# slimgroup/SetIntersectionProjection.jl

Hardware: AMD Instinct MI355X
Metric: PARSDMM iterations/sec (higher is better)
Workload: dtype f32

## Files before the change

### setintersectionprojection.jl_amd/csrc/engine.cpp

```cpp
#include "engine.h"
#include "comm.h"
#include "device_memory.h"
#include "dist_dft.h"
#include "ext_proj.h"
#include "host_prefault.h"
#include "l21_joint.h"
#include "set_config.h"
#include "solve_rules.h"
#include "sparse_granules.h"

#include <algorithm>
#include <array>
#include <chrono>
#include <cmath>
#include <cstdio>
#include <cstdlib>
#include <cstring>
#include <limits>
#include <thread>
#include <exception>

namespace sipx {

const LaunchObserver*& launch_observer() {
// ... 1720 lines not shown
        B.in_rhs = behind ? 0 : 1;
      }
    }
    if (ma.nblk == 0) return false;
    return K<T>::yl_multi(stream_, G_, ma, true);
  }
  static bool sweep_eligible(const SetState<T>& s) {
    return s.owned && !s.custom && !s.ext_kind && !s.dist_ext &&
           (s.prox == PX_BOUNDS || s.prox == PX_L1 || s.prox == PX_PROX_L1 || s.prox == PX_L2 || s.prox == PX_ANNULUS || s.prox == PX_DIST);
  }

  void spec_fill(const LockStep& L, size_t j, long long fseg, long long rank_off, double cap_max, SpecPackArgs<T>& pk, SpecFinishArgs<T>& fa) {
    const SetState<T>& s = sets_[L.tp[j]];
    ProjScalars<T>* ps = L.feas_ps ? s.psf : s.ps;
    SpecPackSet<T>& P = pk.s[j];
    P.ps = ps; P.partials = s.ptmp; P.maxpart = s.mpart; P.compact = s.cbuf;
    P.seg = fbuf_ + rank_off + (long long)j * fseg;
    P.is_l1 = s.prox == PX_L1 ? 1 : 0;
    SpecFinishSet<T>& F = fa.s[j];
    F.ps = ps;
    F.da = DecideArgs{L.args[j].prox, (L.args[j].flags & F_NOSPEC) ? 1 : 0, (double)L.args[j].plo, (double)L.args[j].phi, cap_max, s.Mtrue};
    F.reg = stage_ + j * L.RS;
    F.fseg0 = fbuf_ + (long long)j * fseg;
    F.compact = s.cbuf; F.partials = s.ptmp; F.radius = L.args[j].phi;
    F.host_want = L.ctl[j].host_want; F.verdict = L.ctl[j].verdict;
  }

  void spec_exchange_searches(LockStep& L, int it) {
    const std::vector<int>& tp = L.tp;
    const long long fseg = hooks_.fcap + fast_hdr<T>();
    const long long fchunk = (long long)tp.size() * fseg;
    const unsigned seq = ++spec_seq_ & 0x3fffffffu;
    for (size_t j = 0; j < tp.size(); ++j) {
      L.ctl[j].verdict = (unsigned*)hverd_ + tp[j];
      L.ctl[j].seq = seq;
    }
    if ((int)tp.size() <= SPEC_MAX_SETS) {
      SpecPackArgs<T> pk;
      SpecFinishArgs<T> fa;
      pk.nsets = fa.nsets = (int)tp.size();
      pk.cap = hooks_.fcap;
      fa.world = comm_->world; fa.fchunk = fchunk; fa.seq = seq;
      if (!L.feas_ps && !L.v_is_s && Gr_.n[0] % 4 == 0) {
        LeanMulti<T> lm;
        lm.ns = 0;
        std::vector<size_t> who;
        for (size_t j = 0; j < tp.size() && lm.ns < LEAN_MAX; ++j) {
// ... 149 lines not shown
        LeanSet<T>& S = G.s[G.ns++];
        S.a = L.args[j]; S.a.ps = ps; S.ps = ps; S.compact = s.cbuf; S.partials = s.ptmp; S.maxpart = s.mpart;
      }
      return G;
    };
    std::vector<size_t> all(tp.size());
    for (size_t j = 0; j < tp.size(); ++j) all[j] = j;
    std::vector<size_t> l1s;
    for (size_t j = 0; vec && j < tp.size(); ++j)
      if (sets_[tp[j]].prox == PX_L1 && !(L.args[j].flags & F_NOSPEC)) l1s.push_back(j);
    for (size_t k = 0; k < l1s.size(); k += LEAN_MAX) K<T>::lean_multi(stream_, Gr_, group(l1s, k));
    if (vec && env_knobs().pass_multi) {
      for (size_t k = 0; k < all.size(); k += LEAN_MAX) K<T>::pass_multi(0, stream_, Gr_, group(all, k), L.v_is_s);
    } else {
      for (size_t j : l1s) {
        L.ctl[j].lean_done = 1;
        L.ctl[j].lean_known = feas_ps ? 0 : ((hlean_[tp[j]] >> 16) & 1);
      }
      for (size_t j = 0; j < tp.size(); ++j) search_stage(13, stream_, L, j);
    }
    SpecPackArgs<T> pk;
    SpecFinishArgs<T> fa;
    pk.nsets = fa.nsets = (int)tp.size();
    pk.local = fa.local = 1;
    pk.cap = 0;
    fa.world = 1; fa.fchunk = (long long)tp.size() * fseg; fa.seq = seq;
    for (size_t j = 0; j < tp.size(); ++j) spec_fill(L, j, fseg, 0, 0.0, pk, fa);
    K<T>::spec_sums_pack(stream_, pk);
    K<T>::spec_finish(stream_, fa);
    std::vector<size_t> fb;
    bool refine = false;
    for (size_t j = 0; j < tp.size(); ++j) {
      const unsigned w = wait_verdict(hverd_ + tp[j], seq);
      batch_searches_ += 1;
      if (!(w & 1u)) continue;
      batch_fallbacks_ += 1;
      if (env_knobs().trace_searches)
        std::fprintf(stderr, "[sipx search] search %lld (set %d%s): fallback%s\n", batch_searches_, tp[j], feas_ps ? ", feasibility" : "", (w & 2u) ? " with refinement" : "");
      fb.push_back(j);
      refine |= (w & 2u) != 0;
    }
    const bool spec_debug = env_knobs().spec_debug;
    if (spec_debug && !feas_ps) {
      std::fprintf(stderr, "[sipx spec] batched chain, search seq %u\n", seq);
      for (size_t j = 0; j < tp.size(); ++j) dump_ps(tp[j], stage_ + j * L.RS);
    }
    if (fb.empty()) return;
    auto tail = [&](int stage) {
      for (size_t j : fb) {
        SetState<T>& s = sets_[tp[j]];
        K<T>::search_tail(stage, stream_, L.args[j], feas_ps ? s.psf : s.ps, s.ptmp, s.mpart, s.cbuf, s.Mtrue, L.ctl[j], stage_ + j * L.RS);
// ... 1127 lines not shown
    }
    o += ", \"rank_route\": {\"calls\": " + std::to_string(rc[0]) + ", \"warm_started_subspace\": " + std::to_string(rc[1]) +
         ", \"full_decomposition\": " + std::to_string(rc[2]) + ", \"products_with_gram\": " + std::to_string(rc[3]) + "}";
    long long fc[4] = {0, 0, 0, 0};
    for (const auto& st : sets_) {
      if (!st.ext || st.ext_kind != EXT_L21_SEG) continue;
      long long c[4];
      st.ext->route_counts(c);
      fc[0] += c[0]; fc[1] = std::max(fc[1], c[1]); fc[3] += c[3];
    }
    o += ", \"l21_frames\": {\"passes_total\": " + std::to_string(fc[0]) + ", \"passes_max\": " + std::to_string(fc[1]) +
         ", \"frames\": " + std::to_string(fc[3]) + "}}";
    if (!peek) start_stats(enable);
    return o.c_str();
  }
  double stat_pair_overhead_ms() const { return stat_pair_ms_; }

  void debug_proj(int set, int which, double* o) override {
    need_final();
    for (int k = 0; k < 16; ++k) o[k] = 0;
    if (set < 0 || set >= p_n_) throw std::runtime_error("set index out of range");
    const ProjScalars<T>* d = (which & 1) ? sets_[set].psf : sets_[set].ps;
    if (!d) return;
    ProjScalars<T> h;
    SIPX_HIP(hipStreamSynchronize(stream_));
    SIPX_HIP(hipMemcpy(&h, d, sizeof(h), hipMemcpyDeviceToHost));
    o[0] = h.need; o[1] = h.theta; o[2] = h.theta_prev; o[3] = h.hw; o[4] = h.spec_lo; o[5] = h.spec_hi; o[6] = h.lo;
    o[7] = h.hi; o[8] = h.asum; o[9] = h.vmax; o[10] = h.dbg[0]; o[11] = h.dbg[1]; o[12] = h.dbg[2]; o[13] = h.dbg[3];
    o[14] = h.refine;
    o[15] = h.lean + 2 * h.dbg_sampled;
    if (which & 2) { o[4] = h.samp_theta; o[5] = h.samp_lo; o[6] = h.samp_hi; o[7] = h.samp_c; }
  }

  void* stream() override { return (void*)stream_; }
  void* dev_rhs() override { return rhs_; }
  void* dev_x() override { return x_; }
  void get_rhs(void* out) override {
    need_final();
    if (slab_local_ && comm_->world > 1) throw std::runtime_error("a slab-decomposed context holds its planes of rhs only");
    SIPX_HIP(hipStreamSynchronize(stream_));
    SIPX_HIP(hipMemcpy(out, rhs_, Nx_ * sizeof(T), hipMemcpyDeviceToHost));
  }

 private:
  struct KSample { int kid; double bytes_survey, bytes_moved; };
  struct KAgg { long long launches = 0, noops = 0; double ms = 0, bytes_survey = 0, bytes_moved = 0; };
// ... 658 lines not shown
  bool lean_multi_ = false;
  bool head_done_ = false;
  int merged_nslots_ = 0;
  int sums_flags_ = 0;
  volatile unsigned long long* ticket_ = nullptr;
  unsigned cg_seq_ = 0;
  bool slab_req_ = false, slab_ = false;
  hipStream_t fan_st_ = nullptr;
  hipEvent_t fan_fork_ = nullptr;
  double* fan_ptmp_ = nullptr;
  T *fan_mpart_ = nullptr, *fan_c_ = nullptr;
  long long fan_exchanges_ = 0;
  bool slab_loose_ = false;
  bool slab_full_req_ = false, slab_local_ = false;
  std::string selftest_ = "none", mapped_why_;
  double* agree_buf_ = nullptr;
  bool selftest_mapped_failed_ = false, selftest_alltoall_failed_ = false;
  std::string a2a_why_;
  long long wlo_ = 0, whi_ = 0;
  Grid Gr_, Gyl_;
  ChainHooks hooks_;
  T* gbuf_ = nullptr;
  double *stage_ = nullptr, *sstage_ = nullptr;
  const ChainHooks* hooks() const { return slab_ ? &hooks_ : nullptr; }
  double obj_ss_ = 0, evo_ss_ = 0, xx_ss_ = 0;
  bool have_log_sums_ = false;
  hipEvent_t cg_ev_[2] = {nullptr, nullptr};
  std::vector<hipEvent_t> stat_ev_;
  std::vector<KSample> samples_;
  std::vector<size_t> open_;
  int stats_mode_ = 0;
  LaunchObserver obs_{this, &Engine<T>::obs_begin, &Engine<T>::obs_end};
  std::string stats_json_;
  double stat_pair_ms_ = 0;
};

EngineBase* make_engine(int dtype, int ndim, const int64_t* n, const double* h, int device) {
  const int count = hip_device_count();
  if (device < 0 || device >= count) throw std::runtime_error("libsipx: device index out of range");
  if (dtype == SIPX_F32) return new Engine<float>(ndim, n, h, device);
  if (dtype == SIPX_F64) return new Engine<double>(ndim, n, h, device);
  throw std::runtime_error("dtype must be SIPX_F32 or SIPX_F64");
}

template <typename T>
static void cds_spmv_T(int64_t N, int d, const void* R, const int64_t* off, const void* x, void* y) {
// ... 99 lines not shown
```

### setintersectionprojection.jl_amd/csrc/kernels_proj.hip

```cpp
#include <cstdlib>
#include <cstring>
#include <stdexcept>
#include <string>
#include <type_traits>

#include "sipx_device.h"

namespace sipx {

#if defined(__HIP_DEVICE_COMPILE__) && !defined(__gfx950__)
#error "kernels_proj.hip: the relaxed-atomics hand-offs assume gfx950 (see the comment above); port them to release/acquire first"
#endif

constexpr double L1_CAP = 131072.0;
constexpr int L1_REFINES = 1;
constexpr int L1_REFINES_SLAB = 6;
#ifndef SIPX_SPEC_CAP
#define SIPX_SPEC_CAP 1024
#endif
constexpr int SPEC_CAP = SIPX_SPEC_CAP;
constexpr double L1_HW_MAX = 1e-2;
constexpr double L1_CAPDIV = 64.0;
constexpr int L1_WIN_LO = 3, L1_WIN_HI = 4;
__device__ __forceinline__ double l1_probe_mult(int k) {
// ... 1165 lines not shown
__device__ __forceinline__ DD dd_add(DD a, double b) {
  const double s = a.hi + b, bb = s - a.hi;
  const double e = (a.hi - (s - bb)) + (b - bb);
  return DD{s, a.lo + e};
}
__device__ __forceinline__ DD dd_add(DD a, DD b) {
  const double s = a.hi + b.hi, bb = s - a.hi;
  const double e = (a.hi - (s - bb)) + (b.hi - bb);
  const double lo = (a.lo + b.lo) + e;
  const double hi = s + lo;
  return DD{hi, lo - (hi - s)};
}
__device__ __forceinline__ double shfl_xor_f64(double v, int m) {
  const long long b = __double_as_longlong(v);
  const int lo = __shfl_xor((int)(b & 0xffffffffll), m, 64), hi = __shfl_xor((int)(b >> 32), m, 64);
  return __longlong_as_double(((long long)hi << 32) | (unsigned int)lo);
}
__device__ __forceinline__ DD wave_sum_dd(DD v) {
#pragma unroll
  for (int m = 1; m < 64; m <<= 1) v = dd_add(v, DD{shfl_xor_f64(v.hi, m), shfl_xor_f64(v.lo, m)});
  return v;
}

#ifndef SIPX_SOLVE_NT
#define SIPX_SOLVE_NT 1024
#endif
constexpr int SOLVE_G = 32;
constexpr long long SOLVE_COOP_MIN = 1ll << 17;
static_assert(SOLVE_G <= SIPX_SOLVE_SLOTS, "ProjScalars holds SIPX_SOLVE_SLOTS cooperative slots");

template <typename T>
__device__ void l1_solve_body(ProjScalars<T>* ps, T radius, const T* __restrict__ compact, const double* __restrict__ partials,
                              long long true_len, int* host_want, int only_if_settled,
                              const int G, const int wg) {
  constexpr int NT = SIPX_SOLVE_NT;
  if (only_if_settled && ps->need && !ps->spec_ok) return;
  __shared__ double ssum[NT / 64];
  __shared__ double ssum_lo[NT / 64];
  __shared__ double scnt[NT / 64];
  __shared__ double sh_theta, sh_sa, sh_ca;
  __shared__ int sh_done;
  const int need = ps->need;
  const long long n_all = need ? (long long)ps->n_compact : 0;
  const bool coop = G > 1 && n_all >= SOLVE_COOP_MIN;
  if (!coop && wg != 0) return;
  double theta = 0;
  int iters_done = 0;
  if (need) {
    if (ps->spec_ok) {
      if (threadIdx.x == 0) { sh_sa = ps->s_above; sh_ca = ps->c_above; }
    } else {
      double s = 0, c = 0;
      for (int i = threadIdx.x; i < NB; i += NT) {
        s += partials[(long long)SL_ABOVE_S * NB + i];
        c += partials[(long long)SL_ABOVE_C * NB + i];
      }
      s = wave_sum(s);
      c = wave_sum(c);
      if ((threadIdx.x & 63) == 0) { ssum[threadIdx.x >> 6] = s; scnt[threadIdx.x >> 6] = c; }
      __syncthreads();
      if (threadIdx.x == 0) {
        double S = 0, Cc = 0;
        for (int i = 0; i < NT / 64; ++i) { S += ssum[i]; Cc += scnt[i]; }
        sh_sa = S; sh_ca = Cc;
      }
    }
    __syncthreads();
    const long long nv_all = n_all / 4;
    const long long per = coop ? (nv_all + G - 1) / G : nv_all;
    const long long v0 = coop ? (long long)wg * per : 0, v1 = coop ? (v0 + per < nv_all ? v0 + per : nv_all) : nv_all;
    const bool tail_owner = !coop || wg == G - 1;
    const double sa = sh_sa, ca = sh_ca, b = (double)radius;
    theta = ps->lo;
    double cprev = -1;
    for (int it = 0; it < 200; ++it) {
      DD s = {0.0, 0.0};
      double c = 0;
      {
        const long long nv = v1;
        for (long long i0 = v0 + threadIdx.x; i0 < nv; i0 += 4 * NT) {
          Vec<T, 4> q[4];
#pragma unroll
          for (int u = 0; u < 4; ++u) {
            const long long i = i0 + (long long)u * NT;
            if (i < nv) q[u] = ldv_u<T, 4>(compact + 4 * i);
            else { q[u].v[0] = q[u].v[1] = q[u].v[2] = q[u].v[3] = T(0); }
          }
#pragma unroll
          for (int u = 0; u < 4; ++u)
#pragma unroll
            for (int k = 0; k < 4; ++k) {
              const double av = (double)q[u].v[k];
              if (av > theta) { s = dd_add(s, av); c += 1.0; }
            }
        }
        if (tail_owner)
          for (long long e = 4 * nv_all + threadIdx.x; e < n_all; e += NT) {
            const double av = (double)compact[e];
            if (av > theta) { s = dd_add(s, av); c += 1.0; }
          }
      }
      s = wave_sum_dd(s);
      c = wave_sum(c);
      __syncthreads();
      if ((threadIdx.x & 63) == 0) { ssum[threadIdx.x >> 6] = s.hi; ssum_lo[threadIdx.x >> 6] = s.lo; scnt[threadIdx.x >> 6] = c; }
      __syncthreads();
      if (threadIdx.x == 0) {
        DD Sd = {0.0, 0.0};
        double Cc = 0;
        for (int i = 0; i < NT / 64; ++i) { Sd = dd_add(Sd, DD{ssum[i], ssum_lo[i]}); Cc += scnt[i]; }
        if (coop) {
          const int buf = it & 1;
          __hip_atomic_store(&ps->coop_hi[buf][wg], Sd.hi, __ATOMIC_RELAXED, __HIP_MEMORY_SCOPE_AGENT);
          __hip_atomic_store(&ps->coop_lo[buf][wg], Sd.lo, __ATOMIC_RELAXED, __HIP_MEMORY_SCOPE_AGENT);
          __hip_atomic_store(&ps->coop_c[buf][wg], Cc, __ATOMIC_RELAXED, __HIP_MEMORY_SCOPE_AGENT);
          __hip_atomic_fetch_add(&ps->coop_arrive, 1u, __ATOMIC_RELEASE, __HIP_MEMORY_SCOPE_AGENT);
          const unsigned want = (unsigned)G * (unsigned)(it + 1);
          unsigned spins = 0;
          while (__hip_atomic_load(&ps->coop_arrive, __ATOMIC_ACQUIRE, __HIP_MEMORY_SCOPE_AGENT) < want) {
            if (__hip_atomic_load(&ps->coop_abort, __ATOMIC_RELAXED, __HIP_MEMORY_SCOPE_AGENT)) break;
            if (++spins > 8000000u) {
              __hip_atomic_store(&ps->coop_abort, 1u, __ATOMIC_RELAXED, __HIP_MEMORY_SCOPE_AGENT);
              break;
            }
            __builtin_amdgcn_s_sleep(4);
          }
          Sd = DD{0.0, 0.0};
          Cc = 0;
          for (int k = 0; k < G; ++k) {
            Sd = dd_add(Sd, DD{__hip_atomic_load(&ps->coop_hi[buf][k], __ATOMIC_RELAXED, __HIP_MEMORY_SCOPE_AGENT),
                               __hip_atomic_load(&ps->coop_lo[buf][k], __ATOMIC_RELAXED, __HIP_MEMORY_SCOPE_AGENT)});
            Cc += __hip_atomic_load(&ps->coop_c[buf][k], __ATOMIC_RELAXED, __HIP_MEMORY_SCOPE_AGENT);
          }
        }
        const double S = Sd.hi + Sd.lo;
        const double tot = ca + Cc;
        double tn = theta;
        if (tot > 0) tn = (sa + S - b) / tot;
        sh_done = (Cc == cprev || !(tot > 0)) ? 1 : 0;
        if (coop && __hip_atomic_load(&ps->coop_abort, __ATOMIC_RELAXED, __HIP_MEMORY_SCOPE_AGENT)) sh_done = 1;
        sh_theta = tn > theta ? tn : theta;
        sh_sa = sa; sh_ca = tot;
        scnt[0] = Cc;
      }
      __syncthreads();
      theta = sh_theta;
      cprev = scnt[0];
      iters_done = it + 1;
      if (sh_done) break;
    }
  }
  if (threadIdx.x == 0) {
    if (coop) {
      const unsigned t = __hip_atomic_fetch_add(&ps->coop_finish, 1u, __ATOMIC_ACQ_REL, __HIP_MEMORY_SCOPE_AGENT);
      if (t != (unsigned)G - 1u) return;
      ps->dbg[3] = ps->coop_abort ? -1.0 : 0.0;
      ps->coop_arrive = 0;
      ps->coop_finish = 0;
      ps->coop_abort = 0;
    }
    if (need) {
      if (sh_ca >= (double)true_len && true_len > 1) theta = (ps->asum - (double)ps->vmin - (double)radius) / (double)(true_len - 1);
      const T th = (T)theta;
      ps->theta = th > T(0) ? th : T(0);
      if (ps->gather_overflow) ps->theta = (T)NAN;
    }
    ps->dbg[0] = (double)ps->n_compact; ps->dbg[1] = ps->spec_overflow; ps->dbg[2] = ps->spec_ok;
    ps->dbg[3] = (coop && ps->dbg[3] < 0) ? -1.0 : (double)iters_done;
    ps->lean = (need && theta > 0 && ps->spec_ok && !ps->spec_overflow && sh_ca < (double)true_len) ? 1 : 0;
    ps->want_sample = 0;
    if (need && theta > 0) {
      double hw = ps->hw;
      if (!(ps->theta_prev > 0)) ps->want_sample = 1;
      if (ps->theta_prev > 0) {
        const double d = fabs(theta / ps->theta_prev - 1.0);
        ps->want_sample = (3.0 * d > L1_HW_MAX) ? 1 : 0;
        if (ps->rescaled) ps->resc_bad = d > L1_HW_MAX ? 1 : 0;
        hw = 3.0 * d;
        double hw_floor = 2e-3;
        if (ps->spec_ok && n_all > 0 && ps->hw > 0) {
          const double tgt = fmax(32768.0, (double)true_len / 1024.0);
          hw_floor = ps->hw * tgt / (double)n_all;
          hw_floor = hw_floor < 1e-3 ? 1e-3 : (hw_floor > 4e-3 ? 4e-3 : hw_floor);
        }
        hw = hw < hw_floor ? hw_floor : (hw > L1_HW_MAX ? L1_HW_MAX : hw);
        if (ps->spec_overflow) hw = ps->hw * 0.5;
      }
      ps->hw = hw;
      ps->theta_prev = theta;
      for (int k = 0; k < L1_K; ++k) ps->t[k] = (double)(T)(theta * (1.0 + hw * l1_probe_mult(k)));
      ps->spec_lo = ps->t[L1_WIN_LO];
      ps->spec_hi = ps->t[L1_WIN_HI];
    } else if (ps->theta_prev > 0) {
      for (int k = 0; k < L1_K; ++k) ps->t[k] = (double)(T)(ps->theta_prev * (1.0 + ps->hw * l1_probe_mult(k)));
      ps->spec_lo = ps->t[L1_WIN_LO];
      ps->spec_hi = ps->t[L1_WIN_HI];
    }
    ps->n_compact = 0;
    ps->spec_overflow = 0;
    if (ps->sampled && need && theta > 0) { ps->samp_bias = ps->samp_theta - theta; ps->samp_bias_ok = 1; }
    ps->dbg_sampled = ps->sampled;
    ps->sampled = 0;
    ps->rescaled = 0;
    if (host_want)
      __hip_atomic_store(host_want, ps->want_sample | (ps->rounds_used << 8) | ((ps->lean && ps->spec_hi > ps->spec_lo) ? (1 << 16) : 0), __ATOMIC_RELAXED,
                         __HIP_MEMORY_SCOPE_SYSTEM);
  }
}

template <typename T>
__global__ __launch_bounds__(SIPX_SOLVE_NT) void k_l1_solve(ProjScalars<T>* ps, T radius, const T* __restrict__ compact,
                                                   const double* __restrict__ partials, long long true_len, int* host_want, int only_if_settled) {
  l1_solve_body<T>(ps, radius, compact, partials, true_len, host_want, only_if_settled, (int)gridDim.x,
                   (int)blockIdx.x);
}

constexpr double CARD_CAP = 8192.0;
constexpr int CARD_REFINES = 5;

template <typename T, int STAGE, int SLAB = 0>
__global__ __launch_bounds__(1024) void k_card_decide(const double* __restrict__ partials,
                                                      const T* __restrict__ maxpart, ProjScalars<T>* ps, long long k,
                                                      long long true_len, int world = 1, int rank = 0, double cap_max = CARD_CAP) {
  if (STAGE == 1 && !(ps->need && ps->refine)) return;
  __shared__ double red[PREP_SLOTS];
  __shared__ T smax[16];
  T vmax = T(0);
  if (SLAB != 2) {
    reduce_slots<1024>(partials, red);
    if (STAGE == 0) {
      for (int i = threadIdx.x; i < NB; i += 1024) vmax = maxpart[i] > vmax ? maxpart[i] : vmax;
      vmax = wave_max<T>(vmax);
      if ((threadIdx.x & 63) == 0) smax[threadIdx.x >> 6] = vmax;
    }
  }
  __syncthreads();
  if (threadIdx.x != 0) return;
// ... 270 lines not shown
  if (b < PREP_SLOTS) {
    const double v = block_sum_partials(S.partials + (long long)b * NB);
    if (threadIdx.x == 0) h[b] = v;
    return;
  }
  const long long n = S.is_l1 ? (long long)S.ps->n_compact : 0;
  if (b == PREP_SLOTS) {
    __shared__ T smax[BLOCK / 64], smin[BLOCK / 64];
    T vmax = T(0), vmin = (T)INFINITY;
    for (int i = threadIdx.x; i < NB; i += BLOCK) {
      vmax = S.maxpart[i] > vmax ? S.maxpart[i] : vmax;
      const T mn = S.maxpart[NB + i];
      vmin = (mn > T(0) && mn < vmin) ? mn : vmin;
    }
    vmax = wave_max<T>(vmax);
    vmin = -wave_max<T>(-vmin);
    if ((threadIdx.x & 63) == 0) { smax[threadIdx.x >> 6] = vmax; smin[threadIdx.x >> 6] = vmin; }
    __syncthreads();
    if (threadIdx.x == 0) {
      for (int i = 0; i < BLOCK / 64; ++i) { vmax = smax[i] > vmax ? smax[i] : vmax; vmin = smin[i] < vmin ? smin[i] : vmin; }
      h[FH_OVF] = S.ps->spec_overflow ? 1.0 : 0.0;
      h[FH_MAX] = (double)vmax;
      h[FH_MIN] = (vmin < (T)INFINITY) ? (double)vmin : 0.0;
      h[FH_CNT] = (A.local || n <= A.cap) ? (double)n : -1.0;
    }
    return;
  }
  if (A.local) return;
  const long long m = n <= A.cap ? n : 0;
  for (long long i = (long long)(b - PREP_SLOTS - 1) * BLOCK + threadIdx.x; i < m; i += (long long)SPEC_COPY_WG * BLOCK)
    S.seg[fast_hdr<T>() + i] = S.compact[i];
}
template <typename T>
void K<T>::spec_sums_pack(hipStream_t s, const SpecPackArgs<T>& A) {
  if (A.nsets < 1 || A.nsets > SPEC_MAX_SETS) throw std::runtime_error("spec_sums_pack: set count out of range");
  ObsScope obs_(KID_SLOT_SUMS, s, 0.0);
  hipLaunchKernelGGL((k_spec_sums_pack<T>), dim3(PREP_SLOTS + 1 + (A.local ? 0 : SPEC_COPY_WG), A.nsets), dim3(BLOCK), 0, s, A);
  SIPX_HIP(hipGetLastError());
}

template <typename T>
__global__ __launch_bounds__(SIPX_SOLVE_NT) void k_spec_finish(SpecFinishArgs<T> A) {
  const SpecFinishSet<T>& S = A.s[blockIdx.x];
  ProjScalars<T>* ps = S.ps;
  __shared__ double sreg[PREP_SLOTS + 1 + 2 * SIPX_MAX_WORLD];
  __shared__ double scount;
  const int i = threadIdx.x, world = A.world;
  if (i <= FH_OVF) {
    double v = 0;
    for (int r = 0; r < world; ++r) v += reinterpret_cast<const double*>(S.fseg0 + (long long)r * A.fchunk)[i];
    sreg[i] = v;
  }
  if (i == FH_CNT) {
    double tot = 0;
    bool bad = false;
    for (int r = 0; r < world; ++r) {
      const double* h = reinterpret_cast<const double*>(S.fseg0 + (long long)r * A.fchunk);
      sreg[PREP_SLOTS + 1 + 2 * r] = h[FH_MAX];
      sreg[PREP_SLOTS + 1 + 2 * r + 1] = h[FH_MIN];
      if (h[FH_CNT] < 0) bad = true; else tot += h[FH_CNT];
    }
    scount = bad ? -1.0 : tot;
  }
  __syncthreads();
  if (i == 0 && scount < 0) sreg[FH_OVF] += 1.0;
  __syncthreads();
  if (i < PREP_SLOTS + 1 + 2 * world) S.reg[i] = sreg[i];
  if (i == 0) {
    decide_body<T, 0>(ps, S.da.prox, (T)S.da.pmin, (T)S.da.pmax, S.da.true_len, S.da.nospec, world, S.da.cap_max, sreg);
    const bool settled = !(S.da.prox == PX_L1 && ps->need && !ps->spec_ok);
    if (S.da.prox == PX_L1 && ps->need && ps->spec_ok) ps->n_compact = (unsigned long long)scount;
    ps->gather_overflow = 0;
    const unsigned word = (A.seq << 2) | (settled ? 0u : 1u) | ((!settled && ps->refine) ? 2u : 0u);
    __hip_atomic_store(S.verdict, word, __ATOMIC_RELEASE, __HIP_MEMORY_SCOPE_SYSTEM);
  }
  __threadfence_block();
  __syncthreads();
  if (S.da.prox != PX_L1) return;
  if (ps->need && ps->spec_ok && !A.local) {
    long long off = 0;
    for (int r = 0; r < world; ++r) {
      const T* seg = S.fseg0 + (long long)r * A.fchunk;
      const long long n = (long long)reinterpret_cast<const double*>(seg)[FH_CNT];
      const T* v = seg + fast_hdr<T>();
      for (long long k = threadIdx.x; k < n; k += SIPX_SOLVE_NT) S.compact[off + k] = v[k];
      off += n;
    }
  }
  __threadfence_block();
  __syncthreads();
  l1_solve_body<T>(ps, S.radius, S.compact, S.partials, S.da.true_len, S.host_want, 1, 1, 0);
}
template <typename T>
void K<T>::spec_finish(hipStream_t s, SpecFinishArgs<T>& A) {
  if (A.nsets < 1 || A.nsets > SPEC_MAX_SETS) throw std::runtime_error("spec_finish: set count out of range");
  ObsScope obs_(KID_L1_SOLVE, s, 0.0);
  hipLaunchKernelGGL((k_spec_finish<T>), dim3(A.nsets), dim3(SIPX_SOLVE_NT), 0, s, A);
  SIPX_HIP(hipGetLastError());
}

template <typename T>
__global__ void k_ps_rescale(ProjScalars<T>* ps, double factor) {
  if (!(ps->theta_prev > 0)) return;
  ps->theta_prev *= factor;
  ps->hw = L1_HW_MAX;
  ps->rescaled = 1;
  if (ps->resc_bad) ps->want_sample = 1;
  for (int k = 0; k < L1_K; ++k) ps->t[k] = (double)(T)(ps->theta_prev * (1.0 + ps->hw * l1_probe_mult(k)));
  ps->spec_lo = ps->t[L1_WIN_LO];
  ps->spec_hi = ps->t[L1_WIN_HI];
}
template <typename T>
void K<T>::ps_rescale(hipStream_t s, ProjScalars<T>* ps, double factor) {
  ObsScope obs_(KID_PS_RESCALE, s, 0.0);
// ... 380 lines not shown
```

### setintersectionprojection.jl_amd/csrc/sipx_common.h

```cpp
#pragma once
#include <hip/hip_runtime.h>
#include <stdint.h>
#include <cstdio>

#include "env_knobs.h"

namespace sipx {

constexpr int BLOCK = 256;
constexpr int NB = 2048;
constexpr int NB_7 = 1792;
inline int fit_grid(long long nvec, int cap) {
  const long long need = (nvec + BLOCK - 1) / BLOCK;
  return (int)(need < 1 ? 1 : (need < cap ? need : cap));
}
template <typename... P>
inline bool aligned16(const P*... p) {
  return (((reinterpret_cast<uintptr_t>(p) & 15u) == 0) && ...);
}
inline int launch_blocks(int per_cu) {
  static const int cus = [] {
    int dev = 0, n = 0;
    if (hipGetDevice(&dev) != hipSuccess || hipDeviceGetAttribute(&n, hipDeviceAttributeMultiprocessorCount, dev) != hipSuccess || n <= 0)
      n = 256;
// ... 196 lines not shown
  int flags;
  int vsrc;
  int nblk_or1() const { return nblk > 0 ? nblk : 1; }
};

struct DecideArgs {
  int prox, nospec;
  double pmin, pmax, cap_max;
  long long true_len;
};
constexpr int SPEC_MAX_SETS = 8;
template <typename T>
struct SpecPackSet {
  const ProjScalars<T>* ps;
  const double* partials;
  const T* maxpart;
  const T* compact;
  T* seg;
  int is_l1;
};
template <typename T>
struct SpecPackArgs {
  int nsets;
  int local = 0;
  long long cap;
  SpecPackSet<T> s[SPEC_MAX_SETS];
};
template <typename T>
struct SpecFinishSet {
  ProjScalars<T>* ps;
  DecideArgs da;
  double* reg;
  const T* fseg0;
  T* compact;
  const double* partials;
  T radius;
  int* host_want;
  unsigned* verdict;
};
template <typename T>
struct SpecFinishArgs {
  int local = 0;
  int nsets, world;
  long long fchunk;
  unsigned seq;
  SpecFinishSet<T> s[SPEC_MAX_SETS];
};

template <typename T>
struct SampleSet {
  SetArgs<T> a;
  ProjScalars<T>* ps;
  double* partials;
  double* reg;
  long long true_len;
};
template <typename T>
struct SampleMulti {
// ... 258 lines not shown
```

### setintersectionprojection.jl_amd/host.py

```python
from __future__ import annotations

import ctypes as C
import os
from dataclasses import dataclass, field
from typing import Any, List, Optional, Sequence, Tuple

import numpy as np

LIB_PATH = os.environ.get("SIPX_LIBRARY") or os.path.join(os.path.dirname(os.path.abspath(__file__)), "libsipx.so")

EXPORTED_SYMBOLS = [
    "sipx_last_error", "sipx_create", "sipx_destroy", "sipx_add_set", "sipx_set_rows", "sipx_num_terms",
    "sipx_finalize", "sipx_rhs_compose", "sipx_argmin_x", "sipx_update_y_l", "sipx_log_scalars",
    "sipx_adapt_rho_gamma", "sipx_q_update", "sipx_download", "sipx_parsdmm", "sipx_parsdmm_begin",
    "sipx_parsdmm_steps", "sipx_cds_spmv",
    "sipx_apply_op", "sipx_apply_op_adj", "sipx_project", "sipx_get_Q", "sipx_time_spmv", "sipx_kernel_stats",
    "sipx_debug_proj", "sipx_resample_nn", "sipx_set_q_mode", "sipx_apply_Q",
    "sipx_stream",
    "sipx_dev_rhs", "sipx_dev_x", "sipx_set_owned", "sipx_get_rhs", "sipx_prox_l2s",
    "sipx_rccl_unique_id", "sipx_set_comm_rccl", "sipx_set_comm", "sipx_slab", "sipx_warm_start_from", "sipx_set_decomp",
    "sipx_kernel_stats_json", "sipx_comm_info", "sipx_device_bytes", "sipx_reset", "sipx_dwt",
    "sipx_learn_observations",
    "sipx_finalize_dev", "sipx_reset_dev", "sipx_download_dev", "sipx_set_caller_stream", "sipx_io_bytes",
    "sipx_q_terms", "sipx_set_data", "sipx_set_data_dev", "sipx_segment_norms", "sipx_segment_norms_dev",
# ... 1021 lines not shown
    def get_Q(self):
        d = C.c_int()
        offs = np.zeros(32, np.int64)
        _chk(lib().sipx_get_Q(self.h, None, offs.ctypes.data_as(C.c_void_p), C.byref(d)))
        Q = np.empty((self.Nx, d.value), self.TF, order="F")
        _chk(lib().sipx_get_Q(self.h, _ptr(Q), offs.ctypes.data_as(C.c_void_p), C.byref(d)))
        return Q, offs[:d.value].copy()

    def time_spmv(self, reps=20):
        ms = C.c_double()
        _chk(lib().sipx_time_spmv(self.h, int(reps), C.byref(ms)))
        return ms.value

    def debug_proj(self, set_index: int, which: int = 0):
        out = np.zeros(16)
        _chk(lib().sipx_debug_proj(self.h, int(set_index), int(which), out.ctypes.data_as(C.c_void_p)))
        keys = ("need", "theta", "theta_prev", "hw", "spec_lo", "spec_hi", "lo", "hi", "asum", "vmax", "gathered",
                "overflow", "spec_ok", "michelot_its", "refine", "lean")
        d = dict(zip(keys, out))
        d["sampled"] = float(int(d["lean"]) >> 1)
        d["lean"] = float(int(d["lean"]) & 1)
        return d

    def kernel_stats(self, enable):
        n, ms = C.c_int64(), C.c_double()
        _chk(lib().sipx_kernel_stats(self.h, int(enable), C.byref(n), C.byref(ms)))
        return n.value, ms.value

    def kernel_stats_all(self, enable):
        import json
        txt = lib().sipx_kernel_stats_json(self.h, int(enable))
        if txt is None:
            raise SipxError(lib().sipx_last_error().decode())
        return json.loads(txt.decode())

    def device_bytes(self):
        a, b, c = C.c_int64(), C.c_int64(), C.c_int64()
        _chk(lib().sipx_device_bytes(self.h, C.byref(a), C.byref(b), C.byref(c)))
        return {"context": a.value, "device_used": b.value, "device_total": c.value}

    def comm_info(self):
        n, r, d = C.c_int(), C.c_int(), C.c_int()
        ver = C.create_string_buffer(64)
        _chk(lib().sipx_comm_info(self.h, C.byref(n), C.byref(r), ver, 64, C.byref(d)))
        return {"nranks": n.value, "rank": r.value, "version": ver.value.decode(), "decomposition": "slab" if d.value == 1 else "sets"}

# ... 741 lines not shown
```

Measured before the change: 869.0.

## Fold local spec sums into spec_finish and stage solver scalars in LDS

On the single-rank batched search path, the separate spec_sums_pack launch is removed. spec_finish now reduces the partial sums and min/max itself in a new local header routine. The ProjScalars block is copied into shared memory at kernel entry and written back at exit, and the L1 threshold solve keeps the first chunk of compact values in registers across its iterations. Together these aim to cut a kernel launch, repeated global scalar traffic and repeated reloads, at the cost of higher register and LDS pressure. Optional phase-stamp instrumentation and a debug readout of the search sums are also added.

New measurement: 868.8 (median of 2 runs). Within noise of the previous version (-0.0%).

```diff
diff --git a/setintersectionprojection.jl_amd/csrc/engine.cpp b/setintersectionprojection.jl_amd/csrc/engine.cpp
--- a/setintersectionprojection.jl_amd/csrc/engine.cpp
+++ b/setintersectionprojection.jl_amd/csrc/engine.cpp
@@ -1766,7 +1766,7 @@
     F.da = DecideArgs{L.args[j].prox, (L.args[j].flags & F_NOSPEC) ? 1 : 0, (double)L.args[j].plo, (double)L.args[j].phi, cap_max, s.Mtrue};
     F.reg = stage_ + j * L.RS;
     F.fseg0 = fbuf_ + (long long)j * fseg;
-    F.compact = s.cbuf; F.partials = s.ptmp; F.radius = L.args[j].phi;
+    F.compact = s.cbuf; F.partials = s.ptmp; F.maxpart = s.mpart; F.is_l1 = P.is_l1; F.radius = L.args[j].phi;
     F.host_want = L.ctl[j].host_want; F.verdict = L.ctl[j].verdict;
   }
 
@@ -1962,11 +1962,12 @@
     SpecPackArgs<T> pk;
     SpecFinishArgs<T> fa;
     pk.nsets = fa.nsets = (int)tp.size();
-    pk.local = fa.local = 1;
+    fa.local = 1;
     pk.cap = 0;
     fa.world = 1; fa.fchunk = (long long)tp.size() * fseg; fa.seq = seq;
     for (size_t j = 0; j < tp.size(); ++j) spec_fill(L, j, fseg, 0, 0.0, pk, fa);
-    K<T>::spec_sums_pack(stream_, pk);
+    if (last_reg_.size() < sets_.size()) last_reg_.resize(sets_.size(), nullptr);
+    for (size_t j = 0; j < tp.size(); ++j) last_reg_[tp[j]] = fa.s[j].reg;
     K<T>::spec_finish(stream_, fa);
     std::vector<size_t> fb;
     bool refine = false;
@@ -3140,6 +3141,18 @@
     if (set < 0 || set >= p_n_) throw std::runtime_error("set index out of range");
     const ProjScalars<T>* d = (which & 1) ? sets_[set].psf : sets_[set].ps;
     if (!d) return;
+    if (which & 12) {
+      constexpr int NR = PREP_SLOTS + 3;
+      const double* reg = ((size_t)set < last_reg_.size() && last_reg_[set])
+                              ? last_reg_[set]
+                              : reinterpret_cast<const double*>(reinterpret_cast<const char*>(d) + offsetof(ProjScalars<T>, red));
+      double r[NR];
+      SIPX_HIP(hipStreamSynchronize(stream_));
+      SIPX_HIP(hipMemcpy(r, reg, sizeof(r), hipMemcpyDeviceToHost));
+      const int k0 = (which & 4) ? 0 : 16;
+      for (int k = 0; k < 16 && k0 + k < NR; ++k) o[k] = r[k0 + k];
+      return;
+    }
     ProjScalars<T> h;
     SIPX_HIP(hipStreamSynchronize(stream_));
     SIPX_HIP(hipMemcpy(&h, d, sizeof(h), hipMemcpyDeviceToHost));
@@ -3844,6 +3857,7 @@
   ChainHooks hooks_;
   T* gbuf_ = nullptr;
   double *stage_ = nullptr, *sstage_ = nullptr;
+  std::vector<const double*> last_reg_;
   const ChainHooks* hooks() const { return slab_ ? &hooks_ : nullptr; }
   double obj_ss_ = 0, evo_ss_ = 0, xx_ss_ = 0;
   bool have_log_sums_ = false;
diff --git a/setintersectionprojection.jl_amd/csrc/kernels_proj.hip b/setintersectionprojection.jl_amd/csrc/kernels_proj.hip
--- a/setintersectionprojection.jl_amd/csrc/kernels_proj.hip
+++ b/setintersectionprojection.jl_amd/csrc/kernels_proj.hip
@@ -1211,6 +1211,53 @@
   return v;
 }
 
+enum { PH_ENTRY = 0, PH_SUMS = 1, PH_DECIDED = 2, PH_LOADED = 3, PH_SWEEP = 4, PH_SOLVED = 5, PH_TAIL = 6 };
+#ifdef SIPX_PHASE_STAMPS
+constexpr int STAMP_REC = 32, STAMP_MAX = 4096;
+__device__ unsigned long long g_stamp[STAMP_MAX * STAMP_REC];
+__device__ unsigned g_stamp_n;
+__shared__ unsigned long long* sh_stamp_rec;
+__shared__ int sh_stamp_k;
+__device__ __forceinline__ void stamp_mark(int phase) {
+  if (threadIdx.x != 0 || !sh_stamp_rec || sh_stamp_k >= STAMP_REC - 4) return;
+  sh_stamp_rec[4 + sh_stamp_k++] = ((unsigned long long)phase << 56) | (wall_clock64() & 0x00ffffffffffffffull);
+}
+__device__ __forceinline__ void stamp_begin(int kernel, bool active) {
+  if (threadIdx.x != 0) return;
+  sh_stamp_rec = nullptr;
+  sh_stamp_k = 0;
+  if (active) {
+    const unsigned r = atomicAdd(&g_stamp_n, 1u);
+    if (r < (unsigned)STAMP_MAX) {
+      sh_stamp_rec = g_stamp + (size_t)r * STAMP_REC;
+      sh_stamp_rec[0] = (unsigned long long)kernel;
+      sh_stamp_rec[1] = sh_stamp_rec[2] = sh_stamp_rec[3] = 0;
+    }
+  }
+  stamp_mark(PH_ENTRY);
+}
+__device__ __forceinline__ void stamp_end(double gathered, int sweeps) {
+  if (threadIdx.x != 0 || !sh_stamp_rec) return;
+  sh_stamp_rec[1] = (unsigned long long)gathered;
+  sh_stamp_rec[2] = (unsigned long long)sweeps;
+  sh_stamp_rec[3] = (unsigned long long)sh_stamp_k;
+}
+extern "C" int sipx_phase_stamps(unsigned long long* out, int max_rec) {
+  unsigned n = 0, zero = 0;
+  if (hipDeviceSynchronize() != hipSuccess) return -1;
+  if (hipMemcpyFromSymbol(&n, HIP_SYMBOL(g_stamp_n), sizeof(n)) != hipSuccess) return -1;
+  n = n > (unsigned)STAMP_MAX ? (unsigned)STAMP_MAX : n;
+  n = n > (unsigned)max_rec ? (unsigned)max_rec : n;
+  if (n && hipMemcpyFromSymbol(out, HIP_SYMBOL(g_stamp), (size_t)n * STAMP_REC * sizeof(unsigned long long)) != hipSuccess) return -1;
+  if (hipMemcpyToSymbol(HIP_SYMBOL(g_stamp_n), &zero, sizeof(zero)) != hipSuccess) return -1;
+  return (int)n;
+}
+#else
+__device__ __forceinline__ void stamp_mark(int) {}
+__device__ __forceinline__ void stamp_begin(int, bool) {}
+__device__ __forceinline__ void stamp_end(double, int) {}
+#endif
+
 #ifndef SIPX_SOLVE_NT
 #define SIPX_SOLVE_NT 1024
 #endif
@@ -1219,22 +1266,71 @@
 static_assert(SOLVE_G <= SIPX_SOLVE_SLOTS, "ProjScalars holds SIPX_SOLVE_SLOTS cooperative slots");
 
 template <typename T>
-__device__ void l1_solve_body(ProjScalars<T>* ps, T radius, const T* __restrict__ compact, const double* __restrict__ partials,
+struct PsStaged {
+  static constexpr int A_END = (int)(offsetof(ProjScalars<T>, coop_hi) / 4);
+  static constexpr int B_BEG = (int)(offsetof(ProjScalars<T>, rescaled) / 4);
+  static constexpr int B_END = (int)(sizeof(ProjScalars<T>) / 4);
+  static_assert(offsetof(ProjScalars<T>, coop_hi) % 4 == 0 && offsetof(ProjScalars<T>, rescaled) % 4 == 0 && sizeof(ProjScalars<T>) % 4 == 0,
+                "staged in 4-byte words");
+  static_assert(offsetof(ProjScalars<T>, coop_hi) < offsetof(ProjScalars<T>, hist) && offsetof(ProjScalars<T>, samp_ticket) < offsetof(ProjScalars<T>, rescaled),
+                "the fields other workgroups touch lie between the two staged ranges");
+};
+template <typename T>
+__device__ __forceinline__ unsigned ps_stage_issue(const ProjScalars<T>* ps, int& w) {
+  using R = PsStaged<T>;
+  constexpr int COUNT = R::A_END + (R::B_END - R::B_BEG);
+  static_assert(COUNT <= SIPX_SOLVE_NT, "one staged word per thread");
+  const int i = (int)threadIdx.x < COUNT ? (int)threadIdx.x : COUNT - 1;
+  w = i < R::A_END ? i : i - R::A_END + R::B_BEG;
+  return reinterpret_cast<const unsigned*>(ps)[w];
+}
+template <typename T>
+__device__ __forceinline__ void ps_stage_commit(ProjScalars<T>* L, unsigned word, int w) {
+  using R = PsStaged<T>;
+  if ((int)threadIdx.x < R::A_END + (R::B_END - R::B_BEG)) reinterpret_cast<unsigned*>(L)[w] = word;
+}
+template <typename T>
+__device__ __forceinline__ void ps_stage_out(ProjScalars<T>* ps, const ProjScalars<T>* L) {
+  using R = PsStaged<T>;
+  const unsigned* src = reinterpret_cast<const unsigned*>(L);
+  unsigned* dst = reinterpret_cast<unsigned*>(ps);
+  for (int i = threadIdx.x; i < R::A_END + (R::B_END - R::B_BEG); i += blockDim.x) {
+    const int w = i < R::A_END ? i : i - R::A_END + R::B_BEG;
+    dst[w] = src[w];
+  }
+}
+
+#ifndef SIPX_SOLVE_REG_V
+#define SIPX_SOLVE_REG_V 16
+#endif
+template <typename T>
+struct SolveRegs {
+  static constexpr int V = SIPX_SOLVE_REG_V;
+};
+template <>
+struct SolveRegs<double> {
+  static constexpr int V = SIPX_SOLVE_REG_V / 2;
+};
+static_assert(SIPX_SOLVE_REG_V % 8 == 0, "the streamed rounds behind the registers start on a multiple of four vectors");
+
+template <typename T>
+__device__ __forceinline__ bool l1_solve_core(ProjScalars<T>* gps, ProjScalars<T>* ps, T radius, const T* __restrict__ compact, const double* __restrict__ partials,
                               long long true_len, int* host_want, int only_if_settled,
                               const int G, const int wg) {
   constexpr int NT = SIPX_SOLVE_NT;
-  if (only_if_settled && ps->need && !ps->spec_ok) return;
+  if (only_if_settled && ps->need && !ps->spec_ok) return false;
   __shared__ double ssum[NT / 64];
   __shared__ double ssum_lo[NT / 64];
   __shared__ double scnt[NT / 64];
   __shared__ double sh_theta, sh_sa, sh_ca;
-  __shared__ int sh_done;
+  __shared__ int sh_done, sh_wrote;
   const int need = ps->need;
   const long long n_all = need ? (long long)ps->n_compact : 0;
   const bool coop = G > 1 && n_all >= SOLVE_COOP_MIN;
-  if (!coop && wg != 0) return;
+  if (!coop && wg != 0) return false;
   double theta = 0;
   int iters_done = 0;
+  if (threadIdx.x == 0) sh_wrote = 1;
   if (need) {
     if (ps->spec_ok) {
       if (threadIdx.x == 0) { sh_sa = ps->s_above; sh_ca = ps->c_above; }
@@ -1262,12 +1358,38 @@
     const double sa = sh_sa, ca = sh_ca, b = (double)radius;
     theta = ps->lo;
     double cprev = -1;
+    constexpr int RV = SolveRegs<T>::V;
+    const long long vreg = v1 - v0 < (long long)RV * NT ? v1 - v0 : (long long)RV * NT;
+    const int nslot = (int)((vreg + NT - 1) / NT);
+    Vec<T, 4> q[RV];
+#pragma unroll
+    for (int u = 0; u < RV; ++u) {
+      const long long i = v0 + threadIdx.x + (long long)u * NT;
+      if (i < v0 + vreg) q[u] = ldv_u<T, 4>(compact + 4 * i);
+      else { q[u].v[0] = q[u].v[1] = q[u].v[2] = q[u].v[3] = T(0); }
+    }
+    T qt = T(0);
+    if (tail_owner && 4 * nv_all + threadIdx.x < n_all) qt = compact[4 * nv_all + threadIdx.x];
+#ifdef SIPX_PHASE_STAMPS
+    __builtin_amdgcn_s_waitcnt(0);
+    stamp_mark(PH_LOADED);
+#endif
     for (int it = 0; it < 200; ++it) {
       DD s = {0.0, 0.0};
       double c = 0;
+#pragma unroll
+      for (int u = 0; u < RV; ++u)
+        if (u < nslot) {
+#pragma unroll
+          for (int k = 0; k < 4; ++k) {
+            asm volatile("" : "+v"(q[u].v[k]));
+            const double av = (double)q[u].v[k];
+            if (av > theta) { s = dd_add(s, av); c += 1.0; }
+          }
+        }
       {
         const long long nv = v1;
-        for (long long i0 = v0 + threadIdx.x; i0 < nv; i0 += 4 * NT) {
+        for (long long i0 = v0 + (long long)RV * NT + threadIdx.x; i0 < nv; i0 += 4 * NT) {
           Vec<T, 4> q[4];
 #pragma unroll
           for (int u = 0; u < 4; ++u) {
@@ -1283,11 +1405,8 @@
               if (av > theta) { s = dd_add(s, av); c += 1.0; }
             }
         }
-        if (tail_owner)
-          for (long long e = 4 * nv_all + threadIdx.x; e < n_all; e += NT) {
-            const double av = (double)compact[e];
-            if (av > theta) { s = dd_add(s, av); c += 1.0; }
-          }
+        const double av = (double)qt;
+        if (av > theta) { s = dd_add(s, av); c += 1.0; }
       }
       s = wave_sum_dd(s);
       c = wave_sum(c);
@@ -1300,16 +1419,16 @@
         for (int i = 0; i < NT / 64; ++i) { Sd = dd_add(Sd, DD{ssum[i], ssum_lo[i]}); Cc += scnt[i]; }
         if (coop) {
           const int buf = it & 1;
-          __hip_atomic_store(&ps->coop_hi[buf][wg], Sd.hi, __ATOMIC_RELAXED, __HIP_MEMORY_SCOPE_AGENT);
-          __hip_atomic_store(&ps->coop_lo[buf][wg], Sd.lo, __ATOMIC_RELAXED, __HIP_MEMORY_SCOPE_AGENT);
-          __hip_atomic_store(&ps->coop_c[buf][wg], Cc, __ATOMIC_RELAXED, __HIP_MEMORY_SCOPE_AGENT);
-          __hip_atomic_fetch_add(&ps->coop_arrive, 1u, __ATOMIC_RELEASE, __HIP_MEMORY_SCOPE_AGENT);
+          __hip_atomic_store(&gps->coop_hi[buf][wg], Sd.hi, __ATOMIC_RELAXED, __HIP_MEMORY_SCOPE_AGENT);
+          __hip_atomic_store(&gps->coop_lo[buf][wg], Sd.lo, __ATOMIC_RELAXED, __HIP_MEMORY_SCOPE_AGENT);
+          __hip_atomic_store(&gps->coop_c[buf][wg], Cc, __ATOMIC_RELAXED, __HIP_MEMORY_SCOPE_AGENT);
+          __hip_atomic_fetch_add(&gps->coop_arrive, 1u, __ATOMIC_RELEASE, __HIP_MEMORY_SCOPE_AGENT);
           const unsigned want = (unsigned)G * (unsigned)(it + 1);
           unsigned spins = 0;
-          while (__hip_atomic_load(&ps->coop_arrive, __ATOMIC_ACQUIRE, __HIP_MEMORY_SCOPE_AGENT) < want) {
-            if (__hip_atomic_load(&ps->coop_abort, __ATOMIC_RELAXED, __HIP_MEMORY_SCOPE_AGENT)) break;
+          while (__hip_atomic_load(&gps->coop_arrive, __ATOMIC_ACQUIRE, __HIP_MEMORY_SCOPE_AGENT) < want) {
+            if (__hip_atomic_load(&gps->coop_abort, __ATOMIC_RELAXED, __HIP_MEMORY_SCOPE_AGENT)) break;
             if (++spins > 8000000u) {
-              __hip_atomic_store(&ps->coop_abort, 1u, __ATOMIC_RELAXED, __HIP_MEMORY_SCOPE_AGENT);
+              __hip_atomic_store(&gps->coop_abort, 1u, __ATOMIC_RELAXED, __HIP_MEMORY_SCOPE_AGENT);
               break;
             }
             __builtin_amdgcn_s_sleep(4);
@@ -1317,9 +1436,9 @@
           Sd = DD{0.0, 0.0};
           Cc = 0;
           for (int k = 0; k < G; ++k) {
-            Sd = dd_add(Sd, DD{__hip_atomic_load(&ps->coop_hi[buf][k], __ATOMIC_RELAXED, __HIP_MEMORY_SCOPE_AGENT),
-                               __hip_atomic_load(&ps->coop_lo[buf][k], __ATOMIC_RELAXED, __HIP_MEMORY_SCOPE_AGENT)});
-            Cc += __hip_atomic_load(&ps->coop_c[buf][k], __ATOMIC_RELAXED, __HIP_MEMORY_SCOPE_AGENT);
+            Sd = dd_add(Sd, DD{__hip_atomic_load(&gps->coop_hi[buf][k], __ATOMIC_RELAXED, __HIP_MEMORY_SCOPE_AGENT),
+                               __hip_atomic_load(&gps->coop_lo[buf][k], __ATOMIC_RELAXED, __HIP_MEMORY_SCOPE_AGENT)});
+            Cc += __hip_atomic_load(&gps->coop_c[buf][k], __ATOMIC_RELAXED, __HIP_MEMORY_SCOPE_AGENT);
           }
         }
         const double S = Sd.hi + Sd.lo;
@@ -1327,10 +1446,11 @@
         double tn = theta;
         if (tot > 0) tn = (sa + S - b) / tot;
         sh_done = (Cc == cprev || !(tot > 0)) ? 1 : 0;
-        if (coop && __hip_atomic_load(&ps->coop_abort, __ATOMIC_RELAXED, __HIP_MEMORY_SCOPE_AGENT)) sh_done = 1;
+        if (coop && __hip_atomic_load(&gps->coop_abort, __ATOMIC_RELAXED, __HIP_MEMORY_SCOPE_AGENT)) sh_done = 1;
         sh_theta = tn > theta ? tn : theta;
         sh_sa = sa; sh_ca = tot;
         scnt[0] = Cc;
+        stamp_mark(PH_SWEEP);
       }
       __syncthreads();
       theta = sh_theta;
@@ -1339,15 +1459,21 @@
       if (sh_done) break;
     }
   }
-  if (threadIdx.x == 0) {
-    if (coop) {
-      const unsigned t = __hip_atomic_fetch_add(&ps->coop_finish, 1u, __ATOMIC_ACQ_REL, __HIP_MEMORY_SCOPE_AGENT);
-      if (t != (unsigned)G - 1u) return;
-      ps->dbg[3] = ps->coop_abort ? -1.0 : 0.0;
-      ps->coop_arrive = 0;
-      ps->coop_finish = 0;
-      ps->coop_abort = 0;
-    }
+  stamp_mark(PH_SOLVED);
+  bool last = threadIdx.x == 0;
+  if (last && coop) {
+    const unsigned t = __hip_atomic_fetch_add(&gps->coop_finish, 1u, __ATOMIC_ACQ_REL, __HIP_MEMORY_SCOPE_AGENT);
+    if (t != (unsigned)G - 1u) {
+      last = false;
+      sh_wrote = 0;
+    } else {
+      ps->dbg[3] = gps->coop_abort ? -1.0 : 0.0;
+      gps->coop_arrive = 0;
+      gps->coop_finish = 0;
+      gps->coop_abort = 0;
+    }
+  }
+  if (last) {
     if (need) {
       if (sh_ca >= (double)true_len && true_len > 1) theta = (ps->asum - (double)ps->vmin - (double)radius) / (double)(true_len - 1);
       const T th = (T)theta;
@@ -1394,14 +1520,24 @@
     if (host_want)
       __hip_atomic_store(host_want, ps->want_sample | (ps->rounds_used << 8) | ((ps->lean && ps->spec_hi > ps->spec_lo) ? (1 << 16) : 0), __ATOMIC_RELAXED,
                          __HIP_MEMORY_SCOPE_SYSTEM);
-  }
+    stamp_mark(PH_TAIL);
+    stamp_end(ps->dbg[0], iters_done);
+  }
+  __syncthreads();
+  return sh_wrote != 0;
 }
 
 template <typename T>
 __global__ __launch_bounds__(SIPX_SOLVE_NT) void k_l1_solve(ProjScalars<T>* ps, T radius, const T* __restrict__ compact,
                                                    const double* __restrict__ partials, long long true_len, int* host_want, int only_if_settled) {
-  l1_solve_body<T>(ps, radius, compact, partials, true_len, host_want, only_if_settled, (int)gridDim.x,
-                   (int)blockIdx.x);
+  __shared__ ProjScalars<T> sps;
+  stamp_begin(1, blockIdx.x == 0);
+  int w;
+  const unsigned word = ps_stage_issue<T>(ps, w);
+  ps_stage_commit<T>(&sps, word, w);
+  __syncthreads();
+  if (l1_solve_core<T>(ps, &sps, radius, compact, partials, true_len, host_want, only_if_settled, (int)gridDim.x, (int)blockIdx.x))
+    ps_stage_out<T>(ps, &sps);
 }
 
 constexpr double CARD_CAP = 8192.0;
@@ -1718,11 +1854,10 @@
       h[FH_OVF] = S.ps->spec_overflow ? 1.0 : 0.0;
       h[FH_MAX] = (double)vmax;
       h[FH_MIN] = (vmin < (T)INFINITY) ? (double)vmin : 0.0;
-      h[FH_CNT] = (A.local || n <= A.cap) ? (double)n : -1.0;
+      h[FH_CNT] = n <= A.cap ? (double)n : -1.0;
     }
     return;
   }
-  if (A.local) return;
   const long long m = n <= A.cap ? n : 0;
   for (long long i = (long long)(b - PREP_SLOTS - 1) * BLOCK + threadIdx.x; i < m; i += (long long)SPEC_COPY_WG * BLOCK)
     S.seg[fast_hdr<T>() + i] = S.compact[i];
@@ -1731,37 +1866,101 @@
 void K<T>::spec_sums_pack(hipStream_t s, const SpecPackArgs<T>& A) {
   if (A.nsets < 1 || A.nsets > SPEC_MAX_SETS) throw std::runtime_error("spec_sums_pack: set count out of range");
   ObsScope obs_(KID_SLOT_SUMS, s, 0.0);
-  hipLaunchKernelGGL((k_spec_sums_pack<T>), dim3(PREP_SLOTS + 1 + (A.local ? 0 : SPEC_COPY_WG), A.nsets), dim3(BLOCK), 0, s, A);
+  hipLaunchKernelGGL((k_spec_sums_pack<T>), dim3(PREP_SLOTS + 1 + SPEC_COPY_WG, A.nsets), dim3(BLOCK), 0, s, A);
   SIPX_HIP(hipGetLastError());
+}
+
+template <typename T>
+__device__ __forceinline__ void spec_local_header(const SpecFinishSet<T>& S, ProjScalars<T>* ps ,
+                                                  unsigned stage_word, int stage_w, double* sreg, double* scount) {
+  constexpr int NT = SIPX_SOLVE_NT, NW = NT / 64, QW = BLOCK / 64, PER = NB / BLOCK, TASKS = PREP_SLOTS * QW, ROUNDS = (TASKS + NW - 1) / NW;
+  static_assert(NB % BLOCK == 0 && NB % NT == 0, "the partial slots divide among the waves");
+  __shared__ double sm[PREP_SLOTS][QW];
+  __shared__ T smax[NW], smin[NW];
+  const int w = threadIdx.x >> 6, lane = threadIdx.x & 63;
+  double ld[ROUNDS][PER];
+#pragma unroll
+  for (int r = 0; r < ROUNDS; ++r) {
+    const int t = w + r * NW < TASKS ? w + r * NW : TASKS - 1;
+    const double* p = S.partials + (long long)(t / QW) * NB + (t % QW) * 64 + lane;
+#pragma unroll
+    for (int j = 0; j < PER; ++j) ld[r][j] = p[j * BLOCK];
+  }
+  T mx[NB / NT], mn[NB / NT];
+#pragma unroll
+  for (int k = 0; k < NB / NT; ++k) { mx[k] = S.maxpart[threadIdx.x + k * NT]; mn[k] = S.maxpart[NB + threadIdx.x + k * NT]; }
+  ps_stage_commit<T>(ps, stage_word, stage_w);
+  T vmax = T(0), vmin = (T)INFINITY;
+#pragma unroll
+  for (int k = 0; k < NB / NT; ++k) {
+    vmax = mx[k] > vmax ? mx[k] : vmax;
+    vmin = (mn[k] > T(0) && mn[k] < vmin) ? mn[k] : vmin;
+  }
+#pragma unroll
+  for (int r = 0; r < ROUNDS; ++r) {
+    const int t = w + r * NW;
+    double a = 0;
+#pragma unroll
+    for (int j = 0; j < PER; ++j) a += ld[r][j];
+    const double tot = wave_sum(a);
+    if (lane == 0 && t < TASKS) sm[t / QW][t % QW] = tot;
+  }
+  vmax = wave_max<T>(vmax);
+  vmin = -wave_max<T>(-vmin);
+  if (lane == 0) { smax[w] = vmax; smin[w] = vmin; }
+  __syncthreads();
+  if (threadIdx.x < PREP_SLOTS) {
+    double s = 0;
+#pragma unroll
+    for (int i = 0; i < QW; ++i) s += sm[threadIdx.x][i];
+    sreg[threadIdx.x] = s;
+  }
+  if (threadIdx.x == PREP_SLOTS) {
+    for (int i = 0; i < NW; ++i) { vmax = smax[i] > vmax ? smax[i] : vmax; vmin = smin[i] < vmin ? smin[i] : vmin; }
+    sreg[FH_OVF] = ps->spec_overflow ? 1.0 : 0.0;
+    sreg[PREP_SLOTS + 1] = (double)vmax;
+    sreg[PREP_SLOTS + 2] = (vmin < (T)INFINITY) ? (double)vmin : 0.0;
+    *scount = S.is_l1 ? (double)ps->n_compact : 0.0;
+  }
 }
 
 template <typename T>
 __global__ __launch_bounds__(SIPX_SOLVE_NT) void k_spec_finish(SpecFinishArgs<T> A) {
   const SpecFinishSet<T>& S = A.s[blockIdx.x];
-  ProjScalars<T>* ps = S.ps;
+  __shared__ ProjScalars<T> sps;
+  ProjScalars<T>* const ps = &sps;
   __shared__ double sreg[PREP_SLOTS + 1 + 2 * SIPX_MAX_WORLD];
   __shared__ double scount;
   const int i = threadIdx.x, world = A.world;
-  if (i <= FH_OVF) {
-    double v = 0;
-    for (int r = 0; r < world; ++r) v += reinterpret_cast<const double*>(S.fseg0 + (long long)r * A.fchunk)[i];
-    sreg[i] = v;
-  }
-  if (i == FH_CNT) {
-    double tot = 0;
-    bool bad = false;
-    for (int r = 0; r < world; ++r) {
-      const double* h = reinterpret_cast<const double*>(S.fseg0 + (long long)r * A.fchunk);
-      sreg[PREP_SLOTS + 1 + 2 * r] = h[FH_MAX];
-      sreg[PREP_SLOTS + 1 + 2 * r + 1] = h[FH_MIN];
-      if (h[FH_CNT] < 0) bad = true; else tot += h[FH_CNT];
-    }
-    scount = bad ? -1.0 : tot;
+  stamp_begin(0, true);
+  int stage_w;
+  const unsigned stage_word = ps_stage_issue<T>(S.ps, stage_w);
+  if (A.local) {
+    spec_local_header<T>(S, ps, stage_word, stage_w, sreg, &scount);
+  } else {
+    ps_stage_commit<T>(ps, stage_word, stage_w);
+    if (i <= FH_OVF) {
+      double v = 0;
+      for (int r = 0; r < world; ++r) v += reinterpret_cast<const double*>(S.fseg0 + (long long)r * A.fchunk)[i];
+      sreg[i] = v;
+    }
+    if (i == FH_CNT) {
+      double tot = 0;
+      bool bad = false;
+      for (int r = 0; r < world; ++r) {
+        const double* h = reinterpret_cast<const double*>(S.fseg0 + (long long)r * A.fchunk);
+        sreg[PREP_SLOTS + 1 + 2 * r] = h[FH_MAX];
+        sreg[PREP_SLOTS + 1 + 2 * r + 1] = h[FH_MIN];
+        if (h[FH_CNT] < 0) bad = true; else tot += h[FH_CNT];
+      }
+      scount = bad ? -1.0 : tot;
+    }
   }
   __syncthreads();
   if (i == 0 && scount < 0) sreg[FH_OVF] += 1.0;
   __syncthreads();
   if (i < PREP_SLOTS + 1 + 2 * world) S.reg[i] = sreg[i];
+  stamp_mark(PH_SUMS);
   if (i == 0) {
     decide_body<T, 0>(ps, S.da.prox, (T)S.da.pmin, (T)S.da.pmax, S.da.true_len, S.da.nospec, world, S.da.cap_max, sreg);
     const bool settled = !(S.da.prox == PX_L1 && ps->need && !ps->spec_ok);
@@ -1769,10 +1968,14 @@
     ps->gather_overflow = 0;
     const unsigned word = (A.seq << 2) | (settled ? 0u : 1u) | ((!settled && ps->refine) ? 2u : 0u);
     __hip_atomic_store(S.verdict, word, __ATOMIC_RELEASE, __HIP_MEMORY_SCOPE_SYSTEM);
+    stamp_mark(PH_DECIDED);
   }
   __threadfence_block();
   __syncthreads();
-  if (S.da.prox != PX_L1) return;
+  if (S.da.prox != PX_L1) {
+    ps_stage_out<T>(S.ps, ps);
+    return;
+  }
   if (ps->need && ps->spec_ok && !A.local) {
     long long off = 0;
     for (int r = 0; r < world; ++r) {
@@ -1785,7 +1988,9 @@
   }
   __threadfence_block();
   __syncthreads();
-  l1_solve_body<T>(ps, S.radius, S.compact, S.partials, S.da.true_len, S.host_want, 1, 1, 0);
+  l1_solve_core<T>(S.ps, ps, S.radius, S.compact, S.partials, S.da.true_len, S.host_want, 1, 1, 0);
+  __syncthreads();
+  ps_stage_out<T>(S.ps, ps);
 }
 template <typename T>
 void K<T>::spec_finish(hipStream_t s, SpecFinishArgs<T>& A) {
diff --git a/setintersectionprojection.jl_amd/csrc/sipx_common.h b/setintersectionprojection.jl_amd/csrc/sipx_common.h
--- a/setintersectionprojection.jl_amd/csrc/sipx_common.h
+++ b/setintersectionprojection.jl_amd/csrc/sipx_common.h
@@ -242,7 +242,6 @@
 template <typename T>
 struct SpecPackArgs {
   int nsets;
-  int local = 0;
   long long cap;
   SpecPackSet<T> s[SPEC_MAX_SETS];
 };
@@ -254,6 +253,8 @@
   const T* fseg0;
   T* compact;
   const double* partials;
+  const T* maxpart;
+  int is_l1;
   T radius;
   int* host_want;
   unsigned* verdict;
diff --git a/setintersectionprojection.jl_amd/host.py b/setintersectionprojection.jl_amd/host.py
--- a/setintersectionprojection.jl_amd/host.py
+++ b/setintersectionprojection.jl_amd/host.py
@@ -1067,6 +1067,12 @@
         d["lean"] = float(int(d["lean"]) & 1)
         return d
 
+    def search_sums(self, set_index: int):
+        a, b = np.zeros(16), np.zeros(16)
+        _chk(lib().sipx_debug_proj(self.h, int(set_index), 4, a.ctypes.data_as(C.c_void_p)))
+        _chk(lib().sipx_debug_proj(self.h, int(set_index), 8, b.ctypes.data_as(C.c_void_p)))
+        return np.concatenate([a, b[:6]])
+
     def kernel_stats(self, enable):
         n, ms = C.c_int64(), C.c_double()
         _chk(lib().sipx_kernel_stats(self.h, int(enable), C.byref(n), C.byref(ms)))
```
